# silence-tang/GaussianIP

Measured on AMD Instinct MI355X. Metric: raster_fwd_bwd_mpix_per_s, higher is better.
Workload: dtype f32; 1 GPU; BASELINE.json configs[1]: 100000 Gaussians (synthetic human surface, SMPL-X-style init), 1024x1024, 4 views per optimizer step, raster forward+backward; gaussians=100000, height=1024, width=1024, prewarm_steps=0, repeats=11, full=False, sh_degree=0, dist_world_size=1, gpus_visible=1, parallelism=1 GPU

## Files before the change

gaussianip_amd/_lib.py:

```python
import ctypes
import os

_HERE = os.path.dirname(os.path.abspath(__file__))
LIB_DIR = os.path.join(_HERE, "lib")

GIP_MAX_VIEWS = 16
GIP_RECORD_BYTES = 64
GIP_PARTIAL_FLOATS = 12
GIP_OK = 0

_vp = ctypes.c_void_p


class GipRasterConfig(ctypes.Structure):
    _fields_ = [("P", ctypes.c_int32), ("V", ctypes.c_int32), ("H", ctypes.c_int32), ("W", ctypes.c_int32),
                ("sh_degree", ctypes.c_int32), ("sh_coeffs", ctypes.c_int32), ("prefiltered", ctypes.c_int32),
                ("debug", ctypes.c_int32), ("scale_modifier", ctypes.c_float),
                ("tanfovx", ctypes.c_float * GIP_MAX_VIEWS), ("tanfovy", ctypes.c_float * GIP_MAX_VIEWS),
                ("capacity", ctypes.c_uint64), ("exact_lists", ctypes.c_int32), ("forward_only", ctypes.c_int32),
                ("sh_scalar", ctypes.c_int32), ("antialiasing", ctypes.c_int32)]


class GipRasterInputs(ctypes.Structure):
    _fields_ = [(n, _vp) for n in ("means3D", "shs", "colors_precomp", "opacities", "scales", "rotations",
                                   "cov3D_precomp", "viewmatrix", "projmatrix", "campos", "bg")]


class GipRasterOutputs(ctypes.Structure):
    _fields_ = [(n, _vp) for n in ("color", "radii", "depth", "alpha", "host_header")]


class GipRasterGradsIn(ctypes.Structure):
    _fields_ = [(n, _vp) for n in ("dL_dcolor", "dL_ddepth", "dL_dalpha", "alpha", "color", "depth")]


class GipRasterGradsOut(ctypes.Structure):
    _fields_ = [(n, _vp) for n in ("dL_dmeans3D", "dL_dmeans2D", "dL_dshs", "dL_dcolors_precomp", "dL_dopacities",
                                   "dL_dscales", "dL_drotations", "dL_dcov3D_precomp")]


class GipRasterStateLayout(ctypes.Structure):
    _fields_ = [(n, ctypes.c_size_t) for n in ("header", "records", "inst_offset", "tile_count", "tile_start",
                                                "tile_cursor", "tile_count_b", "inst_slot", "block_sums", "block_offset", "keys", "n_contrib",
                                                "final_T", "tile_order", "seg_start", "ckpt_start", "seg_tile", "checkpoints", "sh_colors", "total")] + \
               [(n, ctypes.c_uint32) for n in ("tiles_x", "tiles_y", "num_blocks", "reserved")]


_raster = None
_knn = None


def _missing(name):
    return ImportError(
        "gaussianip_amd: %s not found in %s. The HIP extension must be built for gfx950 first "
        "(`python -c 'import __graft_entry__ as g; g.build()'` or `make -C gaussianip_amd/csrc`). "
        "There is no CPU fallback for the product path." % (name, LIB_DIR))


call_counts = {}


class _Counted:

    def __init__(self, lib):
        self._lib = lib
        self._wrapped = {}

    def __getattr__(self, name):
        w = self._wrapped.get(name)
        if w is None:
            fn = getattr(self._lib, name)

            def w(*args, _fn=fn, _name=name):
# ... 251 lines not shown
```

gaussianip_amd/csrc/api.hip:

```cpp
#include <string.h>

#include "gip_internal.h"

static inline size_t align256(size_t x) { return (x + 255) & ~(size_t)255; }

static_assert(offsetof(GipRasterConfig, antialiasing) == 188 && sizeof(GipRasterConfig) == 192, "GipRasterConfig layout");

static bool sh_mfma_path(const GipRasterConfig* c) { return c->sh_coeffs > 0 && c->sh_degree >= 1 && c->V >= 2 && !c->sh_scalar; }

static bool valid_config(const GipRasterConfig* c) {
  if (!c) return false;
  if (c->P < 0 || c->V < 1 || c->V > GIP_MAX_VIEWS || c->H < 1 || c->W < 1) return false;
  if (c->sh_degree < 0 || c->sh_degree > 3) return false;
  if (c->capacity < 1 || c->capacity > 0xfffffff0ull) return false;
  if ((c->H + GIP_TILE - 1) / GIP_TILE > 0xffff || (c->W + GIP_TILE - 1) / GIP_TILE > 0xffff) return false;
  return true;
}

extern "C" int gip_abi_version(void) { return GIP_ABI_VERSION; }

extern "C" const char* gip_status_string(int status) {
  switch (status) {
    case GIP_OK: return "ok";
    case GIP_ERR_BAD_ARGUMENT: return "bad argument (null pointer, or not exactly one of shs/colors_precomp and scales+rotations/cov3D_precomp)";
    case GIP_ERR_BUFFER_TOO_SMALL: return "state or scratch buffer smaller than gip_raster_state_bytes()/gip_raster_scratch_bytes()";
    case GIP_ERR_HIP: return "HIP runtime error";
    case GIP_ERR_UNSUPPORTED: return "unsupported configuration";
    default: return "unknown status";
  }
}

extern "C" int gip_raster_state_layout(const GipRasterConfig* c, GipRasterStateLayout* L) {
  if (!valid_config(c) || !L) return GIP_ERR_BAD_ARGUMENT;
  memset(L, 0, sizeof(*L));
  const size_t P = (size_t)c->P, V = (size_t)c->V;
  L->tiles_x = (uint32_t)((c->W + GIP_TILE - 1) / GIP_TILE);
  L->tiles_y = (uint32_t)((c->H + GIP_TILE - 1) / GIP_TILE);
  L->num_blocks = (uint32_t)((c->P + GIP_BLOCK - 1) / GIP_BLOCK);
  const size_t T = (size_t)L->tiles_x * L->tiles_y, nblk = L->num_blocks;
  size_t off = 0;
  L->header = off;       off = align256(off + sizeof(GipRasterHeader));
  L->tile_count = off;   off = align256(off + V * T * 4);
  L->tile_cursor = off;  off = align256(off + V * T * 4);
  L->tile_count_b = off; off = align256(off + V * T * 4);
  L->tile_start = off;   off = align256(off + (V * T + 1) * 4);
  L->block_sums = off;   off = align256(off + (V * nblk + 1) * 4);
  L->block_offset = off; off = align256(off + (V * nblk + 1) * 4);
  L->records = off;      off = align256(off + V * P * GIP_RECORD_BYTES);
  L->inst_offset = off;  off = align256(off + V * P * 4);
  L->inst_slot = off;    off = align256(off + V * P * GIP_SLOTS * 4);
  L->n_contrib = off;    off = align256(off + V * (size_t)c->H * c->W * 4);
  L->final_T = off;      off = align256(off + V * (size_t)c->H * c->W * 4);
  L->tile_order = off;   off = align256(off + V * T * 4);
  const size_t ckpt_cap = (size_t)c->capacity / GIP_SEGMENT + 1, seg_cap = ckpt_cap + V * T;
  L->seg_start = off;    off = align256(off + (V * T + 1) * 4);
  L->ckpt_start = off;   off = align256(off + (V * T + 1) * 4);
  L->seg_tile = off;     off = align256(off + seg_cap * 4);
  L->checkpoints = off;  off = align256(off + ckpt_cap * GIP_CKPT_FLOATS * 256 * sizeof(float));
  L->keys = off;         off = align256(off + (size_t)c->capacity * 8);
// ... 47 lines not shown
  p.tile_count_b = (uint32_t*)(b + L.tile_count_b);
  p.inst_slot = (uint32_t*)(b + L.inst_slot);
  p.block_sums = (uint32_t*)(b + L.block_sums);
  p.block_offset = (uint32_t*)(b + L.block_offset);
  p.keys = (unsigned long long*)(b + L.keys);
  p.n_contrib = (uint32_t*)(b + L.n_contrib);
  p.final_T = (float*)(b + L.final_T);
  p.tile_order = (uint32_t*)(b + L.tile_order);
  p.seg_start = (uint32_t*)(b + L.seg_start);
  p.ckpt_start = (uint32_t*)(b + L.ckpt_start);
  p.seg_tile = (uint32_t*)(b + L.seg_tile);
  p.checkpoints = (float*)(b + L.checkpoints);
  p.sh_colors = (float*)(b + L.sh_colors);
  p.host_header = nullptr;
  return p;
}

static int check_inputs(const GipRasterConfig* c, const GipRasterInputs* in) {
  if (!in || !in->means3D || !in->opacities || !in->viewmatrix || !in->projmatrix || !in->campos || !in->bg)
    return GIP_ERR_BAD_ARGUMENT;
  if ((in->shs == nullptr) == (in->colors_precomp == nullptr)) return GIP_ERR_BAD_ARGUMENT;
  const bool sr = in->scales != nullptr && in->rotations != nullptr;
  if ((in->scales != nullptr) != (in->rotations != nullptr)) return GIP_ERR_BAD_ARGUMENT;
  if (sr == (in->cov3D_precomp != nullptr)) return GIP_ERR_BAD_ARGUMENT;
  if (in->shs) {
    const int need = (c->sh_degree + 1) * (c->sh_degree + 1);
    if (c->sh_coeffs < need || c->sh_coeffs > 64) return GIP_ERR_BAD_ARGUMENT;
  }
  return GIP_OK;
}

#define HIP_TRY(expr) do { if ((expr) != hipSuccess) return GIP_ERR_HIP; } while (0)

static int after_launch(const GipRasterConfig* c, hipStream_t s) {
  if (hipGetLastError() != hipSuccess) return GIP_ERR_HIP;
  if (c->debug) { if (hipStreamSynchronize(s) != hipSuccess) return GIP_ERR_HIP; }
  return GIP_OK;
}
#define LAUNCH_CHECK() do { int rc_ = after_launch(cfg, s); if (rc_ != GIP_OK) return rc_; } while (0)

namespace {
struct StageTimer {
  hipStream_t s; float* out; hipEvent_t ev[2 * GIP_NUM_STAGES]; bool used[GIP_NUM_STAGES]; bool ok; int created;
  StageTimer(hipStream_t s_, float* out_) : s(s_), out(out_), ok(true), created(0) {
    for (int i = 0; i < GIP_NUM_STAGES; i++) used[i] = false;
    if (out)
      for (int i = 0; i < 2 * GIP_NUM_STAGES && ok; i++) {
        ok = hipEventCreate(&ev[i]) == hipSuccess;
        if (ok) created++;
      }
  }
  void begin(int st) { if (out && ok) { ok = hipEventRecord(ev[2 * st], s) == hipSuccess; used[st] = true; } }
  void end(int st) { if (out && ok) ok = hipEventRecord(ev[2 * st + 1], s) == hipSuccess; }
  int finish() {
    if (!out) return GIP_OK;
    int rc = GIP_OK;
    if (!ok || hipStreamSynchronize(s) != hipSuccess) rc = GIP_ERR_HIP;
    for (int i = 0; i < GIP_NUM_STAGES; i++) {
      if (rc == GIP_OK && used[i]) {
        float ms = 0.f;
        if (hipEventElapsedTime(&ms, ev[2 * i], ev[2 * i + 1]) != hipSuccess) rc = GIP_ERR_HIP;
        out[i] = ms;
      }
    }
    for (int i = 0; i < created; i++) (void)hipEventDestroy(ev[i]);
    return rc;
  }
};
}

static int forward_impl(const GipRasterConfig* cfg, const GipRasterInputs* in, const GipRasterOutputs* out,
                        void* state, size_t state_bytes, void* stream, float* times) {
  if (!valid_config(cfg)) return cfg && (cfg->V > GIP_MAX_VIEWS || cfg->sh_degree > 3) ? GIP_ERR_UNSUPPORTED : GIP_ERR_BAD_ARGUMENT;
  int rc = check_inputs(cfg, in);
  if (rc != GIP_OK) return rc;
  if (!out || !out->color || !out->radii || !out->depth || !out->alpha || !state) return GIP_ERR_BAD_ARGUMENT;
  GipRasterStateLayout L;
  gip_raster_state_layout(cfg, &L);
  if (state_bytes < L.total) return GIP_ERR_BUFFER_TOO_SMALL;
  GipKernelParams kp;
  fill_params(cfg, L, &kp);
  if (!in->shs) kp.sh_mfma = 0;
  GipStatePtrs st = state_ptrs(state, L);
  st.host_header = out->host_header;
  hipStream_t s = (hipStream_t)stream;
  StageTimer tm(s, times);

  tm.begin(GIP_STAGE_CLEAR);
  HIP_TRY(hipMemsetAsync((char*)state + L.header, 0, L.tile_start - L.header, s));
  tm.end(GIP_STAGE_CLEAR);
  if (cfg->P > 0) {
    tm.begin(GIP_STAGE_PREPROCESS);
    if (kp.sh_mfma) gip_launch_sh_forward_mfma(kp, *in, st.sh_colors, s);
    gip_launch_preprocess(kp, *in, out->radii, st, s);
    tm.end(GIP_STAGE_PREPROCESS);
    LAUNCH_CHECK();
  }
  tm.begin(GIP_STAGE_SCAN);
  gip_launch_scan(kp, st, s);
  tm.end(GIP_STAGE_SCAN);
  LAUNCH_CHECK();
  if (cfg->P > 0) {
    tm.begin(GIP_STAGE_SCATTER);
    gip_launch_scatter(kp, st, s);
    tm.end(GIP_STAGE_SCATTER);
    LAUNCH_CHECK();
    tm.begin(GIP_STAGE_TILE_SORT);
    gip_launch_tile_sort(kp, st, s);
    tm.end(GIP_STAGE_TILE_SORT);
    LAUNCH_CHECK();
  }
  tm.begin(GIP_STAGE_RENDER_FWD);
  gip_launch_render_forward(kp, in->bg, st, out->color, out->depth, out->alpha, s);
  tm.end(GIP_STAGE_RENDER_FWD);
  LAUNCH_CHECK();
  return tm.finish();
}

extern "C" int gip_raster_forward(const GipRasterConfig* cfg, const GipRasterInputs* in, const GipRasterOutputs* out,
                                  void* state, size_t state_bytes, void* stream) {
  return forward_impl(cfg, in, out, state, state_bytes, stream, nullptr);
}
extern "C" int gip_raster_forward_profiled(const GipRasterConfig* cfg, const GipRasterInputs* in, const GipRasterOutputs* out,
                                           void* state, size_t state_bytes, void* stream, float* times_ms) {
  if (!times_ms) return GIP_ERR_BAD_ARGUMENT;
  return forward_impl(cfg, in, out, state, state_bytes, stream, times_ms);
}

static int backward_impl(const GipRasterConfig* cfg, const GipRasterInputs* in, const GipRasterGradsIn* gin,
                         const void* state, size_t state_bytes, void* scratch, size_t scratch_bytes,
                         const GipRasterGradsOut* gout, void* stream, float* times) {
  if (!valid_config(cfg)) return GIP_ERR_BAD_ARGUMENT;
  int rc = check_inputs(cfg, in);
  if (rc != GIP_OK) return rc;
  if (!gin || !gin->alpha || !gin->color || !gin->depth || !gout || !state || !scratch) return GIP_ERR_BAD_ARGUMENT;
  if (cfg->forward_only) return GIP_ERR_BAD_ARGUMENT;
  GipRasterStateLayout L;
  gip_raster_state_layout(cfg, &L);
  if (state_bytes < L.total || scratch_bytes < gip_raster_scratch_bytes(cfg)) return GIP_ERR_BUFFER_TOO_SMALL;
  if (cfg->P == 0) return GIP_OK;
  GipKernelParams kp;
  fill_params(cfg, L, &kp);
  if (!in->shs) kp.sh_mfma = 0;
  GipStatePtrs st = state_ptrs(const_cast<void*>(state), L);
  hipStream_t s = (hipStream_t)stream;
  StageTimer tm(s, times);
  tm.begin(GIP_STAGE_RENDER_BWD);
  gip_launch_render_backward(kp, in->bg, st, *gin, (float*)scratch, s);
  tm.end(GIP_STAGE_RENDER_BWD);
  LAUNCH_CHECK();
  tm.begin(GIP_STAGE_GATHER_BWD);
  gip_launch_gather_backward(kp, *in, st, (const float*)scratch, *gout, s);
  if (kp.sh_mfma && (gout->dL_dshs || gout->dL_dmeans3D)) gip_launch_sh_backward_mfma(kp, *in, st, st.sh_colors, *gout, s);
  tm.end(GIP_STAGE_GATHER_BWD);
  LAUNCH_CHECK();
  return tm.finish();
}

extern "C" int gip_raster_backward(const GipRasterConfig* cfg, const GipRasterInputs* in, const GipRasterGradsIn* gin,
// ... 26 lines not shown
```

gaussianip_amd/csrc/binning.hip:

```cpp
#include "gip_internal.h"

#define SCAN_THREADS 1024
#define SCAN_WAVES (SCAN_THREADS / 64)
#define SCAN_CHUNK SCAN_THREADS

__device__ __forceinline__ uint32_t nseg_of(uint32_t count) { return (count + GIP_SEGMENT - 1) / GIP_SEGMENT; }

#define ORDER_CLASSES 6
__device__ __forceinline__ int class_of(uint32_t c) {
  return c >= 2048 ? 0 : c >= 1024 ? 1 : c >= 512 ? 2 : c >= 128 ? 3 : c >= 1 ? 4 : 5;
}

__device__ __forceinline__ uint32_t block_excl_scan(uint32_t v, uint32_t* s_w, uint32_t* total) {
  const int lane = threadIdx.x & 63, wave = threadIdx.x >> 6;
  const uint32_t incl = gip_wave_incl_scan_u32(v);
  __syncthreads();
  if (lane == 63) s_w[wave] = incl;
  __syncthreads();
  uint32_t base = 0, tot = 0;
#pragma unroll
  for (int w = 0; w < SCAN_WAVES; w++) { const uint32_t x = s_w[w]; base += w < wave ? x : 0u; tot += x; }
  *total = tot;
  return base + incl - v;
}

__device__ __forceinline__ uint32_t wave_sum_u32(uint32_t v) {
#pragma unroll
  for (int d = 32; d >= 1; d >>= 1) v += (uint32_t)__shfl_xor((int)v, d, 64);
  return v;
}

__global__ void __launch_bounds__(SCAN_THREADS)
gip_scan_kernel(GipKernelParams kp, const uint32_t* __restrict__ tile_count, const uint32_t* __restrict__ tile_count_b,
                uint32_t* __restrict__ tile_start,
                uint32_t* __restrict__ seg_start, uint32_t* __restrict__ ckpt_start,
                const uint32_t* __restrict__ block_sums, uint32_t* __restrict__ block_offset,
                uint32_t* __restrict__ tile_order, GipRasterHeader* __restrict__ header, uint32_t* __restrict__ host_header) {
  __shared__ uint32_t s_w[SCAN_WAVES];
  __shared__ uint32_t s_acc[2][3 + ORDER_CLASSES];
  __shared__ uint32_t s_max;
  __shared__ uint32_t s_cls[ORDER_CLASSES][SCAN_WAVES];
  const int n = kp.V * kp.T;
  const int n_chunks = (n + SCAN_CHUNK - 1) / SCAN_CHUNK;
  const int tid = threadIdx.x, lane = tid & 63, wave = tid >> 6;
  if ((int)blockIdx.x >= n_chunks) {
    const int nb = kp.V * kp.nblk;
    const int c0 = ((int)blockIdx.x - n_chunks) * SCAN_CHUNK;
    uint32_t before = 0;
    for (int i0 = tid; i0 < c0; i0 += 8 * SCAN_THREADS) {
      uint32_t v8[8];
#pragma unroll
      for (int u = 0; u < 8; u++) { const int i = i0 + u * SCAN_THREADS; v8[u] = i < c0 ? block_sums[i] : 0u; }
#pragma unroll
      for (int u = 0; u < 8; u++) before += v8[u];
    }
    before = wave_sum_u32(before);
    if (tid == 0) s_max = 0u;
    __syncthreads();
    if (lane == 0) atomicAdd(&s_max, before);
    __syncthreads();
    const uint32_t base = s_max;
    const int i = c0 + tid;
    const uint32_t v = i < nb ? block_sums[i] : 0u;
    uint32_t total;
    const uint32_t e = block_excl_scan(v, s_w, &total);
    if (i < nb) block_offset[i] = base + e;
    if (c0 + SCAN_CHUNK >= nb && tid == 0) block_offset[nb] = base + total;
    return;
  }
  const int chunk0 = (int)blockIdx.x * SCAN_CHUNK;
  if (tid < 2 * (3 + ORDER_CLASSES)) (&s_acc[0][0])[tid] = 0u;
  if (tid == 0) s_max = 0u;
  __syncthreads();
  uint32_t b_c = 0, b_s = 0, b_k = 0, t_c = 0, t_s = 0, t_k = 0, mx = 0;
  uint32_t b_cls[ORDER_CLASSES], t_cls[ORDER_CLASSES];
#pragma unroll
  for (int c = 0; c < ORDER_CLASSES; c++) { b_cls[c] = 0; t_cls[c] = 0; }
  for (int i0 = wave * 64; i0 < n; i0 += 8 * SCAN_THREADS) {
    uint32_t va[8], vb[8];
#pragma unroll
    for (int u = 0; u < 8; u++) {
      const int i = i0 + u * SCAN_THREADS + lane;
      va[u] = i < n ? tile_count[i] : 0u;
      vb[u] = i < n ? tile_count_b[i] : 0u;
    }
#pragma unroll
    for (int u = 0; u < 8; u++) {
      const int g0 = i0 + u * SCAN_THREADS;
      if (g0 >= n) break;
      const int i = g0 + lane;
      const uint32_t c = va[u] + vb[u], a = nseg_of(c), k = a ? a - 1 : 0;
      const int cls = i < n ? class_of(c) : -1;
      const bool before = g0 < chunk0;
      t_c += c; t_s += a; t_k += k;
      mx = c > mx ? c : mx;
      if (before) { b_c += c; b_s += a; b_k += k; }
#pragma unroll
      for (int q = 0; q < ORDER_CLASSES; q++) {
        const uint32_t m = (uint32_t)__popcll(__ballot(cls == q));
        t_cls[q] += m;
        if (before) b_cls[q] += m;
      }
    }
  }
  b_c = wave_sum_u32(b_c); b_s = wave_sum_u32(b_s); b_k = wave_sum_u32(b_k);
  t_c = wave_sum_u32(t_c); t_s = wave_sum_u32(t_s); t_k = wave_sum_u32(t_k);
  mx = gip_wave_max_u32(mx);
  if (lane == 0) {
    atomicAdd(&s_acc[0][0], b_c); atomicAdd(&s_acc[0][1], b_s); atomicAdd(&s_acc[0][2], b_k);
    atomicAdd(&s_acc[1][0], t_c); atomicAdd(&s_acc[1][1], t_s); atomicAdd(&s_acc[1][2], t_k);
#pragma unroll
    for (int q = 0; q < ORDER_CLASSES; q++) { atomicAdd(&s_acc[0][3 + q], b_cls[q]); atomicAdd(&s_acc[1][3 + q], t_cls[q]); }
    atomicMax(&s_max, mx);
  }
  __syncthreads();
  const int i = chunk0 + tid;
  uint32_t c = 0;
  if (i < n) c = tile_count[i] + tile_count_b[i];
  const uint32_t a = nseg_of(c), k = a ? a - 1 : 0;
  uint32_t tot;
  const uint32_t e_c = block_excl_scan(c, s_w, &tot);
  const uint32_t e_s = block_excl_scan(a, s_w, &tot);
  const uint32_t e_k = block_excl_scan(k, s_w, &tot);
  if (i < n) {
    tile_start[i] = s_acc[0][0] + e_c;
    seg_start[i] = s_acc[0][1] + e_s;
    ckpt_start[i] = s_acc[0][2] + e_k;
  }
  const int cls = i < n ? class_of(c) : -1;
  uint32_t rank = 0;
#pragma unroll
  for (int q = 0; q < ORDER_CLASSES; q++) {
    const unsigned long long m = __ballot(cls == q);
    if (cls == q) rank = (uint32_t)__popcll(m & ((1ull << lane) - 1ull));
    if (lane == 0) s_cls[q][wave] = (uint32_t)__popcll(m);
  }
  __syncthreads();
  if (cls >= 0) {
    uint32_t pos = rank + s_acc[0][3 + cls];
#pragma unroll
    for (int q = 0; q < ORDER_CLASSES; q++) pos += q < cls ? s_acc[1][3 + q] : 0u;
    for (int w = 0; w < wave; w++) pos += s_cls[cls][w];
    tile_order[pos] = (uint32_t)i;
  }
  if (blockIdx.x == 0 && tid == 0) {
    const uint32_t total = s_acc[1][0];
    tile_start[n] = total; seg_start[n] = s_acc[1][1]; ckpt_start[n] = s_acc[1][2];
    const uint32_t n0 = s_acc[1][3], n1 = s_acc[1][4], n2 = s_acc[1][5], n3 = s_acc[1][6], n4 = s_acc[1][7];
    header->class_end[1] = n0;
    header->class_end[2] = n0 + n1;
    header->class_end[0] = n0 + n1 + n2;
    header->class_end[3] = n0 + n1 + n2 + n3 + n4;
    header->abi_version = GIP_ABI_VERSION;
    header->num_rendered = total;
    header->overflow = (total > kp.capacity) ? 1u : 0u;
    header->max_tile_count = s_max;
    header->num_segments = s_acc[1][1];
    header->num_checkpoints = s_acc[1][2];
    if (host_header) {
      host_header[0] = GIP_ABI_VERSION; host_header[1] = total;
      host_header[2] = (total > kp.capacity) ? 1u : 0u; host_header[3] = s_max;
    }
  }
}

void gip_launch_scan(const GipKernelParams& kp, GipStatePtrs st, hipStream_t s) {
  const int n = kp.V * kp.T, nb = kp.V * kp.nblk;
  const int n_chunks = (n + SCAN_CHUNK - 1) / SCAN_CHUNK, b_chunks = nb > 0 ? (nb + SCAN_CHUNK - 1) / SCAN_CHUNK : 1;
  hipLaunchKernelGGL(gip_scan_kernel, dim3(n_chunks + b_chunks), dim3(SCAN_THREADS), 0, s, kp, st.tile_count, st.tile_count_b, st.tile_start,
                     st.seg_start, st.ckpt_start, st.block_sums, st.block_offset, st.tile_order, st.header, st.host_header);
}

__global__ void __launch_bounds__(GIP_BLOCK)
gip_scatter_kernel(GipKernelParams kp, const GipRecord* __restrict__ records, const uint32_t* __restrict__ tile_start,
                   const uint32_t* __restrict__ tile_count, uint32_t* __restrict__ tile_cursor,
                   const uint32_t* __restrict__ inst_slot, const uint32_t* __restrict__ block_offset,
                   uint32_t* __restrict__ inst_offset, unsigned long long* __restrict__ keys) {
  const int v = blockIdx.y;
  const int idx = blockIdx.x * GIP_BLOCK + threadIdx.x;
  uint32_t tiles = 0, rmin = 0, rmax = 0, dbits = 0, tmask = 0;
  if (idx < kp.P) {
    const uint4* rp = reinterpret_cast<const uint4*>(records + (size_t)v * kp.P + idx);
    const uint4 q0 = rp[0], q1 = rp[1], q3 = rp[3];
    dbits = q0.z; tiles = q1.w; rmin = q3.x; rmax = q3.y; tmask = q3.w;
  }
  __shared__ uint32_t s_wave[4];
  const int lane = threadIdx.x & 63, wave = threadIdx.x >> 6;
  uint32_t incl = gip_wave_incl_scan_u32(tiles);
  if (lane == 63) s_wave[wave] = incl;
  __syncthreads();
  uint32_t base = block_offset[(size_t)v * kp.nblk + blockIdx.x];
  for (int w = 0; w < wave; w++) base += s_wave[w];
  if (idx < kp.P) inst_offset[(size_t)v * kp.P + idx] = base + incl - tiles;
  if (tiles == 0) return;
  const int rminx = rmin & 0xffff, rminy = rmin >> 16, rmaxx = rmax & 0xffff, rmaxy = rmax >> 16;
  const unsigned long long key = ((unsigned long long)dbits << 32) | (uint32_t)idx;
  const size_t tbase = (size_t)v * kp.T;
  const uint4* sp = reinterpret_cast<const uint4*>(inst_slot + ((size_t)v * kp.P + idx) * GIP_SLOTS);
  const uint4 s0 = sp[0];
  uint4 s1 = make_uint4(0, 0, 0, 0);
  if (tiles > 4) s1 = sp[1];
  const uint32_t slots[GIP_SLOTS] = {s0.x, s0.y, s0.z, s0.w, s1.x, s1.y, s1.z, s1.w};
  const int area = (rmaxx - rminx) * (rmaxy - rminy);
  int k = -1, kt = 0;
  for (int ty = rminy; ty < rmaxy; ty++)
    for (int tx = rminx; tx < rmaxx; tx++, kt++) {
      if (!gip_rect_has(tmask, area, kt)) continue;
      k++;
      const size_t t = tbase + ty * kp.tiles_x + tx;
      uint32_t slot;
      if (k < GIP_SLOTS) {
        slot = 0;
#pragma unroll
        for (int kk = 0; kk < GIP_SLOTS; kk++) if (kk == k) slot = slots[kk];
      } else {
        slot = tile_count[t] + atomicAdd(&tile_cursor[t], 1u);
      }
      const uint32_t pos = tile_start[t] + slot;
      if (pos < kp.capacity) keys[pos] = key;
    }
}

void gip_launch_scatter(const GipKernelParams& kp, GipStatePtrs st, hipStream_t s) {
  hipLaunchKernelGGL(gip_scatter_kernel, dim3(kp.nblk, kp.V), dim3(GIP_BLOCK), 0, s, kp, st.records, st.tile_start,
                     st.tile_count, st.tile_cursor, st.inst_slot, st.block_offset, st.inst_offset, st.keys);
}

__device__ __forceinline__ unsigned long long u64min(unsigned long long a, unsigned long long b) { return a < b ? a : b; }
__device__ __forceinline__ unsigned long long u64max(unsigned long long a, unsigned long long b) { return a < b ? b : a; }

template <int MASK>
__device__ __forceinline__ uint32_t lane_xor32(uint32_t x) {
  if constexpr (MASK == 1) return (uint32_t)__builtin_amdgcn_update_dpp(0, (int)x, 0xB1, 0xF, 0xF, false);
  else if constexpr (MASK == 2) return (uint32_t)__builtin_amdgcn_update_dpp(0, (int)x, 0x4E, 0xF, 0xF, false);
  else if constexpr (MASK == 3) return (uint32_t)__builtin_amdgcn_update_dpp(0, (int)x, 0x1B, 0xF, 0xF, false);
  else if constexpr (MASK == 7) return (uint32_t)__builtin_amdgcn_update_dpp(0, (int)x, 0x141, 0xF, 0xF, false);
  else if constexpr (MASK == 15) return (uint32_t)__builtin_amdgcn_update_dpp(0, (int)x, 0x140, 0xF, 0xF, false);
  else if constexpr (MASK == 8) return (uint32_t)__builtin_amdgcn_update_dpp(0, (int)x, 0x128, 0xF, 0xF, false);
  else if constexpr (MASK == 4) {
    const int t = __builtin_amdgcn_update_dpp(0, (int)x, 0x104, 0xF, 0x5, false);
    return (uint32_t)__builtin_amdgcn_update_dpp(t, (int)x, 0x114, 0xF, 0xA, false);
  } else return (uint32_t)__shfl_xor((int)x, MASK, 64);
}
template <int MASK>
__device__ __forceinline__ unsigned long long lane_xor64(unsigned long long x) {
  const uint32_t lo = lane_xor32<MASK>((uint32_t)x), hi = lane_xor32<MASK>((uint32_t)(x >> 32));
  return ((unsigned long long)hi << 32) | lo;
}

template <int R, int MASK>
__device__ __forceinline__ void wave_xor_step(unsigned long long (&v)[R], bool keep_min) {
#pragma unroll
  for (int r = 0; r < R; r++) {
    const unsigned long long p = lane_xor64<MASK>(v[r]);
    v[r] = ((v[r] < p) == keep_min) ? v[r] : p;
  }
}
template <int R, int FROM>
__device__ __forceinline__ void wave_lane_strides(unsigned long long (&v)[R], int lane) {
  if constexpr (FROM >= 32) wave_xor_step<R, 32>(v, !(lane & 32));
  if constexpr (FROM >= 16) wave_xor_step<R, 16>(v, !(lane & 16));
  if constexpr (FROM >= 8) wave_xor_step<R, 8>(v, !(lane & 8));
  if constexpr (FROM >= 4) wave_xor_step<R, 4>(v, !(lane & 4));
  if constexpr (FROM >= 2) wave_xor_step<R, 2>(v, !(lane & 2));
  if constexpr (FROM >= 1) wave_xor_step<R, 1>(v, !(lane & 1));
}
template <int R>
__device__ __forceinline__ void wave_row_strides(unsigned long long (&v)[R], int from) {
#pragma unroll
  for (int jr = R >> 1; jr >= 1; jr >>= 1) {
    if (jr > from) continue;
#pragma unroll
    for (int r = 0; r < R; r++)
      if (!(r & jr)) { const unsigned long long lo = u64min(v[r], v[r + jr]), hi = u64max(v[r], v[r + jr]); v[r] = lo; v[r + jr] = hi; }
  }
}
template <int R, int ROWS>
__device__ __forceinline__ void wave_row_stage(unsigned long long (&v)[R], int lane) {
// ... 304 lines not shown
```

gaussianip_amd/csrc/gip_internal.h:

```cpp
#pragma once
#include <hip/hip_runtime.h>
#include <stdint.h>

#include "../../include/gip_raster.h"

#define GIP_BLOCK 256
#define GIP_WAVE 64
#define GIP_NEAR 0.2f
#define GIP_ALPHA_MIN (1.0f / 255.0f)
#define GIP_ALPHA_MAX 0.99f
#define GIP_T_MIN 0.0001f

struct __attribute__((aligned(16))) GipRecord {
  float x, y, depth, opacity;
  float ca, cb, cc; uint32_t tiles;
  float r, g, b; int32_t radius;
  uint32_t rmin, rmax, clamped, tmask;
};

#define GIP_MASK_TILES 32
__host__ __device__ inline bool gip_rect_has(uint32_t tmask, int area, int k) { return area > GIP_MASK_TILES || ((tmask >> k) & 1u); }
__host__ __device__ inline int gip_rect_rank(uint32_t tmask, int area, int k) {
  return area > GIP_MASK_TILES ? k : __builtin_popcount(tmask & ((1u << k) - 1u));
}

static_assert(sizeof(GipRecord) == GIP_RECORD_BYTES, "record size");

struct GipViewConst {
  float tanfovx, tanfovy, focal_x, focal_y;
};

struct GipKernelParams {
  int P, V, H, W;
  int tiles_x, tiles_y, T;
  int nblk;
  int D, M;
  float scale_modifier;
  uint32_t capacity;
  uint32_t seg_capacity;
  uint32_t ckpt_capacity;
  int exact_lists;
  int forward_only;
  int sh_mfma;
  int antialiasing;
  GipViewConst view[GIP_MAX_VIEWS];
};

struct GipStatePtrs {
  GipRasterHeader* header;
  GipRecord* records;
  uint32_t* inst_offset;
  uint32_t* tile_count;
  uint32_t* tile_start;
  uint32_t* tile_cursor;
  uint32_t* tile_count_b;
  uint32_t* inst_slot;
  uint32_t* block_sums;
  uint32_t* block_offset;
  unsigned long long* keys;
  uint32_t* n_contrib;
  float* final_T;
  uint32_t* tile_order;
  uint32_t* seg_start;
  uint32_t* ckpt_start;
  uint32_t* seg_tile;
  float* checkpoints;
  uint32_t* host_header;
  float* sh_colors;
};

void gip_launch_preprocess(const GipKernelParams& kp, const GipRasterInputs& in, int32_t* radii, GipStatePtrs st, hipStream_t s);
void gip_launch_scan(const GipKernelParams& kp, GipStatePtrs st, hipStream_t s);
void gip_launch_scatter(const GipKernelParams& kp, GipStatePtrs st, hipStream_t s);
void gip_launch_tile_sort(const GipKernelParams& kp, GipStatePtrs st, hipStream_t s);
void gip_launch_render_forward(const GipKernelParams& kp, const float* bg, GipStatePtrs st, float* color, float* depth, float* alpha, hipStream_t s);
void gip_launch_render_backward(const GipKernelParams& kp, const float* bg, GipStatePtrs st, const GipRasterGradsIn& gin, float* partial, hipStream_t s);
void gip_launch_gather_backward(const GipKernelParams& kp, const GipRasterInputs& in, GipStatePtrs st, const float* partial, const GipRasterGradsOut& gout, hipStream_t s);
void gip_launch_sh_forward_mfma(const GipKernelParams& kp, const GipRasterInputs& in, float* sh_colors, hipStream_t s);
void gip_launch_sh_backward_mfma(const GipKernelParams& kp, const GipRasterInputs& in, GipStatePtrs st, const float* sh_gcol, const GipRasterGradsOut& gout, hipStream_t s);
void gip_launch_mark_visible(int P, const float* means3D, const float* view, uint8_t* present, hipStream_t s);

#ifdef __HIPCC__
__device__ __forceinline__ uint32_t gip_wave_incl_scan_u32(uint32_t v) {
  const int lane = threadIdx.x & 63;
#pragma unroll
  for (int d = 1; d < 64; d <<= 1) {
    uint32_t o = __shfl_up(v, d, 64);
    if (lane >= d) v += o;
  }
  return v;
}

__device__ __forceinline__ float gip_wave_sum(float v) {
#pragma unroll
  for (int d = 32; d >= 1; d >>= 1) v += __shfl_xor(v, d, 64);
  return v;
}
__device__ __forceinline__ uint32_t gip_wave_max_u32(uint32_t v) {
#pragma unroll
  for (int d = 32; d >= 1; d >>= 1) { uint32_t o = __shfl_xor(v, d, 64); v = o > v ? o : v; }
  return v;
}
#endif
```

gaussianip_amd/rasterizer.py:

```python
import ctypes
import os
import warnings
from typing import NamedTuple, Optional, Sequence

import torch

from . import _lib


class GaussianRasterizationSettings(NamedTuple):
    image_height: int
    image_width: int
    tanfovx: float
    tanfovy: float
    bg: torch.Tensor
    scale_modifier: float
    viewmatrix: torch.Tensor
    projmatrix: torch.Tensor
    sh_degree: int
    campos: torch.Tensor
    prefiltered: bool
    debug: bool
    antialiasing: bool = False


_MIN_CAPACITY = 1 << 20
_CAPACITY_MARGIN = 65536
_capacity_hint = {}
_pending_checks = []
overflow_events = 0


def _on_overflow():
    return os.environ.get("GIP_RASTER_ON_OVERFLOW", "zero")


def _exact_lists():
    return os.environ.get("GIP_RASTER_EXACT_LISTS", "0") == "1"


def _sh_scalar():
    return os.environ.get("GIP_RASTER_SH_SCALAR", "0") == "1"


def _strict():
    return os.environ.get("GIP_RASTER_SYNC", "0") == "1"


def _hint_key(dev, P, V, H, W):
    return (dev.index if dev.index is not None else torch.cuda.current_device(), P, V, H, W)


def _pick_capacity(key, P, V):
    last = _capacity_hint.get(key)
    if last is None:
        return None
    return int(max(_MIN_CAPACITY, 3 * last + _CAPACITY_MARGIN))


_dummy = {}


def _ptr(t):
    if t is None:
        return None
    if t.numel() == 0:
        d = _dummy.get(t.device)
        if d is None:
            d = _dummy[t.device] = torch.zeros(64, dtype=torch.float32, device=t.device)
        return ctypes.c_void_p(d.data_ptr())
    return ctypes.c_void_p(t.data_ptr())


def _f32c(t, name, shape_last=None):
    if t is None:
        return None
    if not t.is_cuda:
        raise ValueError("%s must be a CUDA/HIP tensor (the rasterizer has no CPU path)" % name)
    if t.dtype != torch.float32 or not t.is_contiguous():
        t = t.float().contiguous()
    return t


class _Plan:
    pass


def _make_config(P, V, H, W, sh_degree, M, scale_modifier, tanfovx, tanfovy, capacity, prefiltered, debug, forward_only=False,
                 antialiasing=False):
    cfg = _lib.GipRasterConfig()
    cfg.P, cfg.V, cfg.H, cfg.W = int(P), int(V), int(H), int(W)
    cfg.sh_degree, cfg.sh_coeffs = int(sh_degree), int(M)
    cfg.prefiltered, cfg.debug = int(bool(prefiltered)), int(bool(debug))
    cfg.scale_modifier = float(scale_modifier)
    for v in range(V):
        cfg.tanfovx[v] = float(tanfovx[v])
        cfg.tanfovy[v] = float(tanfovy[v])
    cfg.capacity = int(capacity)
    cfg.exact_lists = 1 if _exact_lists() else 0
    cfg.forward_only = 1 if forward_only else 0
    cfg.sh_scalar = 1 if _sh_scalar() else 0
    cfg.antialiasing = 1 if antialiasing else 0
    return cfg


def _check(rc, what):
    if rc != _lib.GIP_OK:
        msg = "%s failed: %s (status %d)" % (what, _lib.status_string(rc), rc)
        if rc == 1:
            raise ValueError(msg)
        raise RuntimeError(msg)


def _run_forward(plan, capacity, forward_only=False):
    lib = _lib.raster_lib()
    dev = plan.means3D.device
    cfg = _make_config(plan.P, plan.V, plan.H, plan.W, plan.sh_degree, plan.M, plan.scale_modifier, plan.tanfovx,
                       plan.tanfovy, capacity, plan.prefiltered, plan.debug, forward_only, plan.antialiasing)
    nbytes = lib.gip_raster_state_bytes(ctypes.byref(cfg))
    if nbytes == 0:
        raise ValueError("invalid rasterizer configuration (P=%d V=%d H=%d W=%d sh_degree=%d)" %
                         (plan.P, plan.V, plan.H, plan.W, plan.sh_degree))
    state = torch.empty(nbytes, dtype=torch.uint8, device=dev)
    V, P, H, W = plan.V, plan.P, plan.H, plan.W
    color = torch.empty((V, 3, H, W), dtype=torch.float32, device=dev)
    depth = torch.empty((V, 1, H, W), dtype=torch.float32, device=dev)
    alpha = torch.empty((V, 1, H, W), dtype=torch.float32, device=dev)
    radii = torch.empty((V, P), dtype=torch.int32, device=dev)
    ins = _lib.GipRasterInputs(_ptr(plan.means3D), _ptr(plan.shs), _ptr(plan.colors_precomp), _ptr(plan.opacities),
                               _ptr(plan.scales), _ptr(plan.rotations), _ptr(plan.cov3D_precomp),
                               _ptr(plan.viewmatrix), _ptr(plan.projmatrix), _ptr(plan.campos), _ptr(plan.bg))
    plan.header_slot, plan.host_header = _header_slot()
    outs = _lib.GipRasterOutputs(_ptr(color), _ptr(radii), _ptr(depth), _ptr(alpha),
                                 ctypes.c_void_p(plan.host_header.data_ptr()))
    stream = ctypes.c_void_p(torch.cuda.current_stream(dev).cuda_stream)
    rc = lib.gip_raster_forward(ctypes.byref(cfg), ctypes.byref(ins), ctypes.byref(outs), _ptr(state), nbytes, stream)
    _check(rc, "gip_raster_forward")
    plan.cfg, plan.state, plan.capacity = cfg, state, capacity
    return color, radii, depth, alpha


_HEADER_SLOTS = 64
_header_ring = None
_header_next = 0
_header_owner = [None] * _HEADER_SLOTS


def _header_slot():
    global _header_ring, _header_next
    if _header_ring is None:
        _header_ring = torch.zeros((_HEADER_SLOTS, 16), dtype=torch.int32).pin_memory()
    i = _header_next
    _header_next = (i + 1) % _HEADER_SLOTS
    owner = _header_owner[i]
    if owner is not None and any(e is owner for e in _pending_checks):
# ... 333 lines not shown
```

include/gip_raster.h:

```cpp
#ifndef GIP_RASTER_H
#define GIP_RASTER_H

#include <stddef.h>
#include <stdint.h>

#ifdef __cplusplus
extern "C" {
#endif

#define GIP_ABI_VERSION 4
#define GIP_TILE 16
#define GIP_MAX_VIEWS 16
#define GIP_RECORD_BYTES 64
#define GIP_PARTIAL_FLOATS 12
#ifndef GIP_SEGMENT
#define GIP_SEGMENT 64
#endif
#define GIP_SLOTS 8
#define GIP_CKPT_FLOATS 5

enum {
  GIP_OK = 0,
  GIP_ERR_BAD_ARGUMENT = 1,
  GIP_ERR_BUFFER_TOO_SMALL = 2,
  GIP_ERR_HIP = 3,
  GIP_ERR_UNSUPPORTED = 4
};

typedef struct GipRasterConfig {
  int32_t P;
  int32_t V;
  int32_t H, W;
  int32_t sh_degree;
  int32_t sh_coeffs;
  int32_t prefiltered;
  int32_t debug;
  float scale_modifier;
  float tanfovx[GIP_MAX_VIEWS];
  float tanfovy[GIP_MAX_VIEWS];
  uint64_t capacity;
  int32_t exact_lists;
  int32_t forward_only;
  int32_t sh_scalar;
  int32_t antialiasing;
} GipRasterConfig;

typedef struct GipRasterInputs {
  const float* means3D;
  const float* shs;
  const float* colors_precomp;
  const float* opacities;
  const float* scales;
  const float* rotations;
  const float* cov3D_precomp;
  const float* viewmatrix;
  const float* projmatrix;
  const float* campos;
  const float* bg;
} GipRasterInputs;

typedef struct GipRasterOutputs {
  float*   color;
  int32_t* radii;
  float*   depth;
  float*   alpha;
  uint32_t* host_header;
} GipRasterOutputs;

typedef struct GipRasterGradsIn {
  const float* dL_dcolor;
  const float* dL_ddepth;
  const float* dL_dalpha;
  const float* alpha;
  const float* color;
  const float* depth;
} GipRasterGradsIn;

typedef struct GipRasterGradsOut {
  float* dL_dmeans3D;
  float* dL_dmeans2D;
  float* dL_dshs;
  float* dL_dcolors_precomp;
  float* dL_dopacities;
  float* dL_dscales;
  float* dL_drotations;
  float* dL_dcov3D_precomp;
} GipRasterGradsOut;

typedef struct GipRasterHeader {
  uint32_t abi_version;
  uint32_t num_rendered;
  uint32_t overflow;
  uint32_t max_tile_count;
  uint32_t num_visible;
  uint32_t num_segments;
  uint32_t num_checkpoints;
  uint32_t class_end[4];
// ... 62 lines not shown
```

Baseline: 8484 Mpix/s.

## Fuse tile-count scan into scatter kernel with per-workgroup redundant prefix

Adds a fused scan+scatter kernel. Each workgroup recomputes the per-view tile prefix sum into LDS and its own offsets by re-reading earlier counts, then scatters keys, and the scan jobs are spread across the same grid. This removes one kernel launch and the dependency gap between scan and scatter. In exchange it does redundant global reads per workgroup, bounded by a size heuristic. A split_scan env flag restores the old path.

```diff
diff --git a/gaussianip_amd/_lib.py b/gaussianip_amd/_lib.py
--- a/gaussianip_amd/_lib.py
+++ b/gaussianip_amd/_lib.py
@@ -18,7 +18,7 @@
                 ("debug", ctypes.c_int32), ("scale_modifier", ctypes.c_float),
                 ("tanfovx", ctypes.c_float * GIP_MAX_VIEWS), ("tanfovy", ctypes.c_float * GIP_MAX_VIEWS),
                 ("capacity", ctypes.c_uint64), ("exact_lists", ctypes.c_int32), ("forward_only", ctypes.c_int32),
-                ("sh_scalar", ctypes.c_int32), ("antialiasing", ctypes.c_int32)]
+                ("sh_scalar", ctypes.c_int32), ("antialiasing", ctypes.c_int16), ("split_scan", ctypes.c_int16)]
 
 
 class GipRasterInputs(ctypes.Structure):
diff --git a/gaussianip_amd/csrc/api.hip b/gaussianip_amd/csrc/api.hip
--- a/gaussianip_amd/csrc/api.hip
+++ b/gaussianip_amd/csrc/api.hip
@@ -4,7 +4,8 @@
 
 static inline size_t align256(size_t x) { return (x + 255) & ~(size_t)255; }
 
-static_assert(offsetof(GipRasterConfig, antialiasing) == 188 && sizeof(GipRasterConfig) == 192, "GipRasterConfig layout");
+static_assert(offsetof(GipRasterConfig, antialiasing) == 188 && offsetof(GipRasterConfig, split_scan) == 190 &&
+              sizeof(GipRasterConfig) == 192, "GipRasterConfig layout");
 
 static bool sh_mfma_path(const GipRasterConfig* c) { return c->sh_coeffs > 0 && c->sh_degree >= 1 && c->V >= 2 && !c->sh_scalar; }
 
@@ -158,6 +159,7 @@
   }
   void begin(int st) { if (out && ok) { ok = hipEventRecord(ev[2 * st], s) == hipSuccess; used[st] = true; } }
   void end(int st) { if (out && ok) ok = hipEventRecord(ev[2 * st + 1], s) == hipSuccess; }
+  void none(int st) { if (out) out[st] = 0.f; }
   int finish() {
     if (!out) return GIP_OK;
     int rc = GIP_OK;
@@ -202,15 +204,26 @@
     tm.end(GIP_STAGE_PREPROCESS);
     LAUNCH_CHECK();
   }
-  tm.begin(GIP_STAGE_SCAN);
-  gip_launch_scan(kp, st, s);
-  tm.end(GIP_STAGE_SCAN);
-  LAUNCH_CHECK();
-  if (cfg->P > 0) {
+  const bool fused = !cfg->split_scan && gip_scan_scatter_fits(kp);
+  if (fused) {
+    tm.none(GIP_STAGE_SCAN);
     tm.begin(GIP_STAGE_SCATTER);
-    gip_launch_scatter(kp, st, s);
+    gip_launch_scan_scatter(kp, st, s);
     tm.end(GIP_STAGE_SCATTER);
     LAUNCH_CHECK();
+  } else {
+    tm.begin(GIP_STAGE_SCAN);
+    gip_launch_scan(kp, st, s);
+    tm.end(GIP_STAGE_SCAN);
+    LAUNCH_CHECK();
+  }
+  if (cfg->P > 0) {
+    if (!fused) {
+      tm.begin(GIP_STAGE_SCATTER);
+      gip_launch_scatter(kp, st, s);
+      tm.end(GIP_STAGE_SCATTER);
+      LAUNCH_CHECK();
+    }
     tm.begin(GIP_STAGE_TILE_SORT);
     gip_launch_tile_sort(kp, st, s);
     tm.end(GIP_STAGE_TILE_SORT);
diff --git a/gaussianip_amd/csrc/binning.hip b/gaussianip_amd/csrc/binning.hip
--- a/gaussianip_amd/csrc/binning.hip
+++ b/gaussianip_amd/csrc/binning.hip
@@ -30,29 +30,31 @@
   return v;
 }
 
-__global__ void __launch_bounds__(SCAN_THREADS)
-gip_scan_kernel(GipKernelParams kp, const uint32_t* __restrict__ tile_count, const uint32_t* __restrict__ tile_count_b,
-                uint32_t* __restrict__ tile_start,
-                uint32_t* __restrict__ seg_start, uint32_t* __restrict__ ckpt_start,
-                const uint32_t* __restrict__ block_sums, uint32_t* __restrict__ block_offset,
-                uint32_t* __restrict__ tile_order, GipRasterHeader* __restrict__ header, uint32_t* __restrict__ host_header) {
+template <int U>
+__device__ __forceinline__ void scan_job(const int job, const int V, const int T, const int nblk, const uint32_t capacity, const uint32_t* __restrict__ tile_count,
+                         const uint32_t* __restrict__ tile_count_b, uint32_t* __restrict__ tile_start,
+                         uint32_t* __restrict__ seg_start, uint32_t* __restrict__ ckpt_start,
+                         const uint32_t* __restrict__ block_sums, uint32_t* __restrict__ block_offset,
+                         uint32_t* __restrict__ tile_order, GipRasterHeader* __restrict__ header, uint32_t* __restrict__ host_header) {
   __shared__ uint32_t s_w[SCAN_WAVES];
   __shared__ uint32_t s_acc[2][3 + ORDER_CLASSES];
   __shared__ uint32_t s_max;
   __shared__ uint32_t s_cls[ORDER_CLASSES][SCAN_WAVES];
-  const int n = kp.V * kp.T;
+  const int n = V * T;
   const int n_chunks = (n + SCAN_CHUNK - 1) / SCAN_CHUNK;
-  const int tid = threadIdx.x, lane = tid & 63, wave = tid >> 6;
-  if ((int)blockIdx.x >= n_chunks) {
-    const int nb = kp.V * kp.nblk;
-    const int c0 = ((int)blockIdx.x - n_chunks) * SCAN_CHUNK;
+  const int tid = threadIdx.x, lane = tid & 63;
+  const int wave = __builtin_amdgcn_readfirstlane(tid >> 6);
+  __syncthreads();
+  if (job >= n_chunks) {
+    const int nb = V * nblk;
+    const int c0 = (job - n_chunks) * SCAN_CHUNK;
     uint32_t before = 0;
-    for (int i0 = tid; i0 < c0; i0 += 8 * SCAN_THREADS) {
-      uint32_t v8[8];
-#pragma unroll
-      for (int u = 0; u < 8; u++) { const int i = i0 + u * SCAN_THREADS; v8[u] = i < c0 ? block_sums[i] : 0u; }
-#pragma unroll
-      for (int u = 0; u < 8; u++) before += v8[u];
+    for (int i0 = tid; i0 < c0; i0 += U * SCAN_THREADS) {
+      uint32_t v8[U];
+#pragma unroll
+      for (int u = 0; u < U; u++) { const int i = i0 + u * SCAN_THREADS; v8[u] = i < c0 ? block_sums[i] : 0u; }
+#pragma unroll
+      for (int u = 0; u < U; u++) before += v8[u];
     }
     before = wave_sum_u32(before);
     if (tid == 0) s_max = 0u;
@@ -68,7 +70,7 @@
     if (c0 + SCAN_CHUNK >= nb && tid == 0) block_offset[nb] = base + total;
     return;
   }
-  const int chunk0 = (int)blockIdx.x * SCAN_CHUNK;
+  const int chunk0 = job * SCAN_CHUNK;
   if (tid < 2 * (3 + ORDER_CLASSES)) (&s_acc[0][0])[tid] = 0u;
   if (tid == 0) s_max = 0u;
   __syncthreads();
@@ -76,16 +78,16 @@
   uint32_t b_cls[ORDER_CLASSES], t_cls[ORDER_CLASSES];
 #pragma unroll
   for (int c = 0; c < ORDER_CLASSES; c++) { b_cls[c] = 0; t_cls[c] = 0; }
-  for (int i0 = wave * 64; i0 < n; i0 += 8 * SCAN_THREADS) {
-    uint32_t va[8], vb[8];
-#pragma unroll
-    for (int u = 0; u < 8; u++) {
+  for (int i0 = wave * 64; i0 < n; i0 += U * SCAN_THREADS) {
+    uint32_t va[U], vb[U];
+#pragma unroll
+    for (int u = 0; u < U; u++) {
       const int i = i0 + u * SCAN_THREADS + lane;
       va[u] = i < n ? tile_count[i] : 0u;
       vb[u] = i < n ? tile_count_b[i] : 0u;
     }
 #pragma unroll
-    for (int u = 0; u < 8; u++) {
+    for (int u = 0; u < U; u++) {
       const int g0 = i0 + u * SCAN_THREADS;
       if (g0 >= n) break;
       const int i = g0 + lane;
@@ -143,7 +145,7 @@
     for (int w = 0; w < wave; w++) pos += s_cls[cls][w];
     tile_order[pos] = (uint32_t)i;
   }
-  if (blockIdx.x == 0 && tid == 0) {
+  if (job == 0 && tid == 0) {
     const uint32_t total = s_acc[1][0];
     tile_start[n] = total; seg_start[n] = s_acc[1][1]; ckpt_start[n] = s_acc[1][2];
     const uint32_t n0 = s_acc[1][3], n1 = s_acc[1][4], n2 = s_acc[1][5], n3 = s_acc[1][6], n4 = s_acc[1][7];
@@ -153,46 +155,42 @@
     header->class_end[3] = n0 + n1 + n2 + n3 + n4;
     header->abi_version = GIP_ABI_VERSION;
     header->num_rendered = total;
-    header->overflow = (total > kp.capacity) ? 1u : 0u;
+    header->overflow = (total > capacity) ? 1u : 0u;
     header->max_tile_count = s_max;
     header->num_segments = s_acc[1][1];
     header->num_checkpoints = s_acc[1][2];
     if (host_header) {
       host_header[0] = GIP_ABI_VERSION; host_header[1] = total;
-      host_header[2] = (total > kp.capacity) ? 1u : 0u; host_header[3] = s_max;
-    }
-  }
-}
-
-void gip_launch_scan(const GipKernelParams& kp, GipStatePtrs st, hipStream_t s) {
+      host_header[2] = (total > capacity) ? 1u : 0u; host_header[3] = s_max;
+    }
+  }
+}
+
+__global__ void __launch_bounds__(SCAN_THREADS)
+gip_scan_kernel(GipKernelParams kp, const uint32_t* __restrict__ tile_count, const uint32_t* __restrict__ tile_count_b,
+                uint32_t* __restrict__ tile_start,
+                uint32_t* __restrict__ seg_start, uint32_t* __restrict__ ckpt_start,
+                const uint32_t* __restrict__ block_sums, uint32_t* __restrict__ block_offset,
+                uint32_t* __restrict__ tile_order, GipRasterHeader* __restrict__ header, uint32_t* __restrict__ host_header) {
+  scan_job<8>((int)blockIdx.x, kp.V, kp.T, kp.nblk, kp.capacity, tile_count, tile_count_b, tile_start, seg_start, ckpt_start, block_sums, block_offset, tile_order,
+           header, host_header);
+}
+
+static int scan_jobs(const GipKernelParams& kp) {
   const int n = kp.V * kp.T, nb = kp.V * kp.nblk;
   const int n_chunks = (n + SCAN_CHUNK - 1) / SCAN_CHUNK, b_chunks = nb > 0 ? (nb + SCAN_CHUNK - 1) / SCAN_CHUNK : 1;
-  hipLaunchKernelGGL(gip_scan_kernel, dim3(n_chunks + b_chunks), dim3(SCAN_THREADS), 0, s, kp, st.tile_count, st.tile_count_b, st.tile_start,
+  return n_chunks + b_chunks;
+}
+
+void gip_launch_scan(const GipKernelParams& kp, GipStatePtrs st, hipStream_t s) {
+  hipLaunchKernelGGL(gip_scan_kernel, dim3(scan_jobs(kp)), dim3(SCAN_THREADS), 0, s, kp, st.tile_count, st.tile_count_b, st.tile_start,
                      st.seg_start, st.ckpt_start, st.block_sums, st.block_offset, st.tile_order, st.header, st.host_header);
 }
 
-__global__ void __launch_bounds__(GIP_BLOCK)
-gip_scatter_kernel(GipKernelParams kp, const GipRecord* __restrict__ records, const uint32_t* __restrict__ tile_start,
-                   const uint32_t* __restrict__ tile_count, uint32_t* __restrict__ tile_cursor,
-                   const uint32_t* __restrict__ inst_slot, const uint32_t* __restrict__ block_offset,
-                   uint32_t* __restrict__ inst_offset, unsigned long long* __restrict__ keys) {
-  const int v = blockIdx.y;
-  const int idx = blockIdx.x * GIP_BLOCK + threadIdx.x;
-  uint32_t tiles = 0, rmin = 0, rmax = 0, dbits = 0, tmask = 0;
-  if (idx < kp.P) {
-    const uint4* rp = reinterpret_cast<const uint4*>(records + (size_t)v * kp.P + idx);
-    const uint4 q0 = rp[0], q1 = rp[1], q3 = rp[3];
-    dbits = q0.z; tiles = q1.w; rmin = q3.x; rmax = q3.y; tmask = q3.w;
-  }
-  __shared__ uint32_t s_wave[4];
-  const int lane = threadIdx.x & 63, wave = threadIdx.x >> 6;
-  uint32_t incl = gip_wave_incl_scan_u32(tiles);
-  if (lane == 63) s_wave[wave] = incl;
-  __syncthreads();
-  uint32_t base = block_offset[(size_t)v * kp.nblk + blockIdx.x];
-  for (int w = 0; w < wave; w++) base += s_wave[w];
-  if (idx < kp.P) inst_offset[(size_t)v * kp.P + idx] = base + incl - tiles;
-  if (tiles == 0) return;
+__device__ __forceinline__ void scatter_instances(const GipKernelParams& kp, int v, int idx, uint32_t tiles, uint32_t rmin, uint32_t rmax,
+                                                  uint32_t dbits, uint32_t tmask, const uint32_t* ts, uint32_t ts_base,
+                                                  const uint32_t* __restrict__ tile_count, uint32_t* __restrict__ tile_cursor,
+                                                  const uint32_t* __restrict__ inst_slot, unsigned long long* __restrict__ keys) {
   const int rminx = rmin & 0xffff, rminy = rmin >> 16, rmaxx = rmax & 0xffff, rmaxy = rmax >> 16;
   const unsigned long long key = ((unsigned long long)dbits << 32) | (uint32_t)idx;
   const size_t tbase = (size_t)v * kp.T;
@@ -207,23 +205,149 @@
     for (int tx = rminx; tx < rmaxx; tx++, kt++) {
       if (!gip_rect_has(tmask, area, kt)) continue;
       k++;
-      const size_t t = tbase + ty * kp.tiles_x + tx;
+      const int tv = ty * kp.tiles_x + tx;
       uint32_t slot;
       if (k < GIP_SLOTS) {
         slot = 0;
 #pragma unroll
         for (int kk = 0; kk < GIP_SLOTS; kk++) if (kk == k) slot = slots[kk];
       } else {
-        slot = tile_count[t] + atomicAdd(&tile_cursor[t], 1u);
+        slot = tile_count[tbase + tv] + atomicAdd(&tile_cursor[tbase + tv], 1u);
       }
-      const uint32_t pos = tile_start[t] + slot;
+      const uint32_t pos = ts_base + ts[tv] + slot;
       if (pos < kp.capacity) keys[pos] = key;
     }
+}
+
+__global__ void __launch_bounds__(GIP_BLOCK)
+gip_scatter_kernel(GipKernelParams kp, const GipRecord* __restrict__ records, const uint32_t* __restrict__ tile_start,
+                   const uint32_t* __restrict__ tile_count, uint32_t* __restrict__ tile_cursor,
+                   const uint32_t* __restrict__ inst_slot, const uint32_t* __restrict__ block_offset,
+                   uint32_t* __restrict__ inst_offset, unsigned long long* __restrict__ keys) {
+  const int v = blockIdx.y;
+  const int idx = blockIdx.x * GIP_BLOCK + threadIdx.x;
+  uint32_t tiles = 0, rmin = 0, rmax = 0, dbits = 0, tmask = 0;
+  if (idx < kp.P) {
+    const uint4* rp = reinterpret_cast<const uint4*>(records + (size_t)v * kp.P + idx);
+    const uint4 q0 = rp[0], q1 = rp[1], q3 = rp[3];
+    dbits = q0.z; tiles = q1.w; rmin = q3.x; rmax = q3.y; tmask = q3.w;
+  }
+  __shared__ uint32_t s_wave[4];
+  const int lane = threadIdx.x & 63, wave = threadIdx.x >> 6;
+  uint32_t incl = gip_wave_incl_scan_u32(tiles);
+  if (lane == 63) s_wave[wave] = incl;
+  __syncthreads();
+  uint32_t base = block_offset[(size_t)v * kp.nblk + blockIdx.x];
+  for (int w = 0; w < wave; w++) base += s_wave[w];
+  if (idx < kp.P) inst_offset[(size_t)v * kp.P + idx] = base + incl - tiles;
+  if (tiles == 0) return;
+  scatter_instances(kp, v, idx, tiles, rmin, rmax, dbits, tmask, tile_start + (size_t)v * kp.T, 0u, tile_count, tile_cursor, inst_slot, keys);
 }
 
 void gip_launch_scatter(const GipKernelParams& kp, GipStatePtrs st, hipStream_t s) {
   hipLaunchKernelGGL(gip_scatter_kernel, dim3(kp.nblk, kp.V), dim3(GIP_BLOCK), 0, s, kp, st.records, st.tile_start,
                      st.tile_count, st.tile_cursor, st.inst_slot, st.block_offset, st.inst_offset, st.keys);
+}
+
+#define FUSED_GROUP 4
+#define FUSED_MAX_TILES 16384
+
+__global__ void __launch_bounds__(SCAN_THREADS)
+gip_scan_scatter_kernel(GipKernelParams kp, const GipRecord* __restrict__ records, const uint32_t* __restrict__ tile_count,
+                        const uint32_t* __restrict__ tile_count_b, uint32_t* __restrict__ tile_cursor,
+                        const uint32_t* __restrict__ inst_slot, const uint32_t* __restrict__ block_sums,
+                        uint32_t* __restrict__ inst_offset, unsigned long long* __restrict__ keys,
+                        uint32_t* __restrict__ tile_start, uint32_t* __restrict__ seg_start, uint32_t* __restrict__ ckpt_start,
+                        uint32_t* __restrict__ block_offset, uint32_t* __restrict__ tile_order,
+                        GipRasterHeader* __restrict__ header, uint32_t* __restrict__ host_header) {
+  extern __shared__ uint32_t s_tile[];
+  __shared__ uint32_t s_w[SCAN_WAVES], s_wave[SCAN_WAVES], s_before[2];
+  const int v = blockIdx.y, T = kp.T;
+  const int tid = threadIdx.x, lane = tid & 63, wave = __builtin_amdgcn_readfirstlane(tid >> 6);
+  const int idx = (int)blockIdx.x * SCAN_THREADS + tid;
+  uint32_t tiles = 0, rmin = 0, rmax = 0, dbits = 0, tmask = 0;
+  if (idx < kp.P) {
+    const uint4* rp = reinterpret_cast<const uint4*>(records + (size_t)v * kp.P + idx);
+    const uint4 q0 = rp[0], q1 = rp[1], q3 = rp[3];
+    dbits = q0.z; tiles = q1.w; rmin = q3.x; rmax = q3.y; tmask = q3.w;
+  }
+  if (tid < 2) s_before[tid] = 0u;
+  const uint32_t* tc = tile_count + (size_t)v * T;
+  const uint32_t* tcb = tile_count_b + (size_t)v * T;
+  uint32_t cv[8];
+#pragma unroll
+  for (int u = 0; u < 8; u++) { const int i = u * SCAN_CHUNK + tid; cv[u] = i < T ? tc[i] + tcb[i] : 0u; }
+  const int t_before = v * T, b_before = v * kp.nblk + (int)blockIdx.x * FUSED_GROUP;
+  uint32_t bt = 0, bb = 0;
+  for (int i0 = tid; i0 < t_before; i0 += 4 * SCAN_THREADS) {
+    uint32_t va[4], vb[4];
+#pragma unroll
+    for (int u = 0; u < 4; u++) {
+      const int i = i0 + u * SCAN_THREADS;
+      va[u] = i < t_before ? tile_count[i] : 0u;
+      vb[u] = i < t_before ? tile_count_b[i] : 0u;
+    }
+#pragma unroll
+    for (int u = 0; u < 4; u++) bt += va[u] + vb[u];
+  }
+  for (int i0 = tid; i0 < b_before; i0 += 4 * SCAN_THREADS) {
+    uint32_t v4[4];
+#pragma unroll
+    for (int u = 0; u < 4; u++) { const int i = i0 + u * SCAN_THREADS; v4[u] = i < b_before ? block_sums[i] : 0u; }
+#pragma unroll
+    for (int u = 0; u < 4; u++) bb += v4[u];
+  }
+  bt = wave_sum_u32(bt); bb = wave_sum_u32(bb);
+  const uint32_t incl = gip_wave_incl_scan_u32(tiles);
+  __syncthreads();
+  if (lane == 0) { atomicAdd(&s_before[0], bt); atomicAdd(&s_before[1], bb); }
+  if (lane == 63) s_wave[wave] = incl;
+  uint32_t run = 0;
+  for (int c0 = 0;;) {
+#pragma unroll
+    for (int u = 0; u < 8; u++) {
+      const int g0 = c0 + u * SCAN_CHUNK;
+      if (g0 >= T) break;
+      uint32_t tot;
+      const uint32_t e = block_excl_scan(cv[u], s_w, &tot);
+      if (g0 + tid < T) s_tile[g0 + tid] = run + e;
+      run += tot;
+    }
+    c0 += 8 * SCAN_CHUNK;
+    if (c0 >= T) break;
+#pragma unroll
+    for (int u = 0; u < 8; u++) { const int i = c0 + u * SCAN_CHUNK + tid; cv[u] = i < T ? tc[i] + tcb[i] : 0u; }
+  }
+  __syncthreads();
+  uint32_t base = s_before[1];
+  for (int w = 0; w < wave; w++) base += s_wave[w];
+  if (idx < kp.P) inst_offset[(size_t)v * kp.P + idx] = base + incl - tiles;
+  if (tiles != 0)
+    scatter_instances(kp, v, idx, tiles, rmin, rmax, dbits, tmask, s_tile, s_before[0], tile_count, tile_cursor, inst_slot, keys);
+  const int wgs = (int)(gridDim.x * gridDim.y), n = kp.V * T, nb = kp.V * kp.nblk;
+  const int jobs = (n + SCAN_CHUNK - 1) / SCAN_CHUNK + (nb + SCAN_CHUNK - 1) / SCAN_CHUNK;
+  for (int job = (int)(blockIdx.y * gridDim.x + blockIdx.x); job < jobs; job += wgs)
+    scan_job<4>(job, kp.V, kp.T, kp.nblk, kp.capacity, tile_count, tile_count_b, tile_start, seg_start, ckpt_start, block_sums, block_offset, tile_order, header, host_header);
+}
+
+#define FUSED_MAX_REREAD_BYTES (64ull << 20)
+bool gip_scan_scatter_fits(const GipKernelParams& kp) {
+  if (kp.P <= 0 || kp.T > FUSED_MAX_TILES) return false;
+  const unsigned long long wgs = (unsigned long long)((kp.nblk + FUSED_GROUP - 1) / FUSED_GROUP) * kp.V;
+  const unsigned long long per_wg = 4ull * kp.T * (kp.V + 1) + 2ull * kp.V * kp.nblk;
+  return wgs * per_wg <= FUSED_MAX_REREAD_BYTES;
+}
+
+void gip_launch_scan_scatter(const GipKernelParams& kp, GipStatePtrs st, hipStream_t s) {
+  static bool opted = false;
+  if (!opted) {
+    (void)hipFuncSetAttribute((const void*)gip_scan_scatter_kernel, hipFuncAttributeMaxDynamicSharedMemorySize, FUSED_MAX_TILES * 4);
+    opted = true;
+  }
+  const int groups = (kp.nblk + FUSED_GROUP - 1) / FUSED_GROUP;
+  hipLaunchKernelGGL(gip_scan_scatter_kernel, dim3(groups, kp.V), dim3(SCAN_THREADS), (size_t)kp.T * 4, s, kp, st.records, st.tile_count,
+                     st.tile_count_b, st.tile_cursor, st.inst_slot, st.block_sums, st.inst_offset, st.keys, st.tile_start, st.seg_start,
+                     st.ckpt_start, st.block_offset, st.tile_order, st.header, st.host_header);
 }
 
 __device__ __forceinline__ unsigned long long u64min(unsigned long long a, unsigned long long b) { return a < b ? a : b; }
diff --git a/gaussianip_amd/csrc/gip_internal.h b/gaussianip_amd/csrc/gip_internal.h
--- a/gaussianip_amd/csrc/gip_internal.h
+++ b/gaussianip_amd/csrc/gip_internal.h
@@ -72,6 +72,8 @@
 void gip_launch_preprocess(const GipKernelParams& kp, const GipRasterInputs& in, int32_t* radii, GipStatePtrs st, hipStream_t s);
 void gip_launch_scan(const GipKernelParams& kp, GipStatePtrs st, hipStream_t s);
 void gip_launch_scatter(const GipKernelParams& kp, GipStatePtrs st, hipStream_t s);
+bool gip_scan_scatter_fits(const GipKernelParams& kp);
+void gip_launch_scan_scatter(const GipKernelParams& kp, GipStatePtrs st, hipStream_t s);
 void gip_launch_tile_sort(const GipKernelParams& kp, GipStatePtrs st, hipStream_t s);
 void gip_launch_render_forward(const GipKernelParams& kp, const float* bg, GipStatePtrs st, float* color, float* depth, float* alpha, hipStream_t s);
 void gip_launch_render_backward(const GipKernelParams& kp, const float* bg, GipStatePtrs st, const GipRasterGradsIn& gin, float* partial, hipStream_t s);
diff --git a/gaussianip_amd/rasterizer.py b/gaussianip_amd/rasterizer.py
--- a/gaussianip_amd/rasterizer.py
+++ b/gaussianip_amd/rasterizer.py
@@ -41,6 +41,10 @@
 
 def _sh_scalar():
     return os.environ.get("GIP_RASTER_SH_SCALAR", "0") == "1"
+
+
+def _split_scan():
+    return os.environ.get("GIP_RASTER_SPLIT_SCAN", "0") == "1"
 
 
 def _strict():
@@ -101,6 +105,7 @@
     cfg.forward_only = 1 if forward_only else 0
     cfg.sh_scalar = 1 if _sh_scalar() else 0
     cfg.antialiasing = 1 if antialiasing else 0
+    cfg.split_scan = 1 if _split_scan() else 0
     return cfg
 
 
diff --git a/include/gip_raster.h b/include/gip_raster.h
--- a/include/gip_raster.h
+++ b/include/gip_raster.h
@@ -42,7 +42,8 @@
   int32_t exact_lists;
   int32_t forward_only;
   int32_t sh_scalar;
-  int32_t antialiasing;
+  int16_t antialiasing;
+  int16_t split_scan;
 } GipRasterConfig;
 
 typedef struct GipRasterInputs {
```

After: 8585 Mpix/s (median of 6 runs). +1.2%, better.
